# zraorg/ZRA

Hardware: AMD Instinct MI355X
Metric: compress + RA-decompress GiB/s, 16 GiB @ 64 KiB frames, 1/2/4/8 MI355X (higher is better)
Workload: dtype u8

## Files before the change

zra_amd/csrc/zra_decode.hip:

```cpp
#include "zra_dev.h"
#include "zra_kernels.h"

using namespace zra_dev;

namespace {

constexpr int DEC_THREADS = 64;
constexpr int BATCH = 64;
#ifndef ZRA_XWIN
#define ZRA_XWIN 4032
#endif
constexpr u32 XPRE = 64, XWIN = ZRA_XWIN;
constexpr u32 BLOCK_MAX = 128u << 10;

__constant__ u32 c_ll_base[36] = {0,1,2,3,4,5,6,7,8,9,10,11,12,13,14,15,16,18,20,22,24,28,32,40,48,64,128,256,512,1024,2048,4096,8192,16384,32768,65536};
__constant__ u8 c_ll_bits[36] = {0,0,0,0,0,0,0,0,0,0,0,0,0,0,0,0,1,1,1,1,2,2,3,3,4,6,7,8,9,10,11,12,13,14,15,16};
__constant__ u32 c_ml_base[53] = {3,4,5,6,7,8,9,10,11,12,13,14,15,16,17,18,19,20,21,22,23,24,25,26,27,28,29,30,31,32,33,34,
                                  35,37,39,41,43,47,51,59,67,83,99,131,259,515,1027,2051,4099,8195,16387,32771,65539};
__constant__ u8 c_ml_bits[53] = {0,0,0,0,0,0,0,0,0,0,0,0,0,0,0,0,0,0,0,0,0,0,0,0,0,0,0,0,0,0,0,0,
                                 1,1,1,1,2,2,3,3,4,4,5,7,8,9,10,11,12,13,14,15,16};
__constant__ short c_ll_defnorm[36] = {4,3,2,2,2,2,2,2,2,2,2,2,2,1,1,1,2,2,2,2,2,2,2,2,2,3,2,1,1,1,1,1,-1,-1,-1,-1};
__constant__ short c_ml_defnorm[53] = {1,4,3,2,2,2,2,2,2,1,1,1,1,1,1,1,1,1,1,1,1,1,1,1,1,1,1,1,1,1,1,1,
                                       1,1,1,1,1,1,1,1,1,1,1,1,1,1,-1,-1,-1,-1,-1,-1,-1};
__constant__ short c_of_defnorm[29] = {1,1,1,1,1,1,2,2,2,1,1,1,1,1,1,1,1,1,1,1,1,1,1,1,-1,-1,-1,-1,-1};
__constant__ u16 c_huf_t0[16][2] = {{0,0},{0,0},{38,130},{448,128},{556,128},{714,128},{883,128},{897,128},{926,128},{947,128},{1107,128},{1177,128},{1242,128},{1349,128},{1455,128},{722,128}};
__constant__ u16 c_huf_t1[16][2] = {{1,1},{1,1},{1313,74},{1353,74},{1353,74},{1418,74},{1437,74},{1515,75},{1613,75},{1729,77},{2083,81},{2379,87},{2415,93},{2644,106},{2422,124},{1891,145}};

__device__ __forceinline__ u64 mk_seqsym(u32 baseValue, u32 addBits, u32 nbBits, u32 nextBase) {
  return (u64)baseValue | ((u64)addBits << 32) | ((u64)nbBits << 40) | ((u64)nextBase << 48);
}
__device__ __forceinline__ u32 mk_cell(u32 sym, u32 addBits, u32 nbBits, u32 nextBase) {
  return sym | (addBits << 8) | (nbBits << 16) | (nextBase << 20);
}

#ifdef ZRA_SMALL_PROFILE
__device__ unsigned long long zra_small_prof[64];
extern "C" __attribute__((visibility("default"))) void ZraHipDebugReadSmallProfile(unsigned long long* out16, int reset) {
  (void)hipMemcpyFromSymbol(out16, HIP_SYMBOL(zra_small_prof), sizeof(unsigned long long) * 64);
  if (reset) { unsigned long long z[64] = {0}; (void)hipMemcpyToSymbol(HIP_SYMBOL(zra_small_prof), z, sizeof(z)); }
}
#define SPROF(k) { __builtin_amdgcn_s_waitcnt(0); const u64 n_ = __builtin_amdgcn_s_memtime(); if (lane == 0) atomicAdd(&zra_small_prof[k], n_ - spt_); spt_ = n_; }
#define SPROF_T0 u64 spt_ = __builtin_amdgcn_s_memtime();
#define SPROF_RESET spt_ = __builtin_amdgcn_s_memtime();
#else
#define SPROF(k)
#define SPROF_T0
#define SPROF_RESET
#endif
#ifdef ZRA_SMALL_PROFILE
#define PPROF_T0 u64 ppt_ = __builtin_amdgcn_s_memtime();
#define PPROF(k) if (FUSED) { __builtin_amdgcn_s_waitcnt(0); const u64 n_ = __builtin_amdgcn_s_memtime(); if (lane == 0) atomicAdd(&zra_small_prof[k], n_ - ppt_); ppt_ = n_; }
#define LPROF_T0 u64 lpt_ = __builtin_amdgcn_s_memtime();
#define LPROF(k) { __builtin_amdgcn_s_waitcnt(0); const u64 n_ = __builtin_amdgcn_s_memtime(); atomicAdd(&zra_small_prof[k], n_ - lpt_); lpt_ = n_; }
#else
#define PPROF_T0
// ... 495 lines not shown
        if (have) copy_bytes(a.raOut + q.dstOff, a.out + a.outOff[j] + q.srcOff, have, lane, nthreads);
        if (have < q.len) fill_bytes(a.raOut + q.dstOff + have, 0, q.len - have, lane, nthreads);
      }
    }
  }
}

}

namespace {
template <bool FUSED, bool ALL = false>
__device__ __forceinline__ u32 parse_job(const ZraDecodeArgs& a, const u32 j, ParseShared& S, const int lane, u32* ldsT) {
  u32 outcome = 0;
  {
    const u64 so = a.frameOff[(size_t)j * a.offStride], se = a.frameOff[(size_t)j * a.offStride + 1];
    const u8* const src = a.body + so;
    const bool spanOk = se >= so && se <= a.bodySize;
    const u32 srcSize = spanOk ? (u32)(se - so) : 0u;
    u8* const dst = a.out + a.outOff[j];
    const u32 dstCap = a.outCap[j];
    const u32 limit = a.limit ? a.limit[j] : 0xFFFFFFFFu;
    ZraDecFrame* const F = &a.frames[j];
    u32 nBlk = 0; bool bail = false;
    const u32* prevT[3] = {nullptr, nullptr, nullptr};

    auto stage = [&](u8* w, u32 pos) -> u32 {
      const u32 avail = pos < srcSize ? min(srcSize - pos, STAGE_BYTES) : 0u;
      const u32 at = 8u * (u32)lane;
      u64 v = 0;
      if (at + 8 <= avail) v = ld64(src + pos + at);
      else for (u32 k = 0; at + k < avail && k < 8; k++) v |= (u64)src[pos + at + k] << (8 * k);
      *(u64*)(w + at) = v;
      if (lane < 2) *(u64*)(w + STAGE_BYTES + 8 * lane) = 0;
      return avail;
    };
    PPROF_T0
    const u32 startPos = a.round == 0 ? 0u : F->blkPos;
    const u32 staged0 = stage(S.w0, startPos);

    if (lane == 0) {
      S.err = 0; S.frameEnd = 0; S.winPos = startPos; S.winLen = staged0;
      if (a.round == 0) {
        S.produced = 0; S.hufValid = 0; S.llValid = S.mlValid = S.ofValid = 0; S.ofShare = 0;
        S.rep[0] = 1; S.rep[1] = 4; S.rep[2] = 8;
      }
    }
    wsync();
// ... 140 lines not shown
        if (S.err) { S.lateErr = S.err; S.err = 0; S.nbSeq = 0; S.seqTables = 0; }
        if (S.alloc && S.nbSeq) {
          const u64 take = ((u64)S.nbSeq + 3) & ~3ull;
          const u64 at = atomicAdd((unsigned long long*)&a.counters[ZRA_DC_SEQCUR], (unsigned long long)take);
          if (at + take > a.seqCap) S.alloc = 0;
          S.seqBase = at;
        }
      }
      wsync();
      if (ALL && (!S.alloc || nBlk >= a.bpf)) { bail = true; break; }
      if (!S.alloc) {
        if (lane == 0) {
          save_persistent(S.hdrPos, produced0, hv0, hmb0, hns0, hx20);
          if (!FUSED) a.nextActive[atomicAdd(&a.counters[ZRA_DC_NNEXT], 1u)] = j;
        }
        handed = true; outcome = 2;
        wsync();
        break;
      }

      PPROF(10)
      const u32 nbSeq = S.nbSeq, regen = S.litRegen;
      const size_t jb = ALL ? (size_t)j * a.bpf + nBlk : (size_t)j;
      u32* const T = ALL ? a.blkTables + jb * ZRA_DEC_TBL_WORDS : a.tables + (size_t)j * ZRA_DEC_TBL_WORDS;
      if (S.seqTables) {
        for (int kind = 0; kind < 3; kind++) {
          const int k = kind == 0 ? 0 : kind == 1 ? 2 : 1;
          const u32 mode = k == 0 ? (S.seqModes >> 6) : k == 2 ? ((S.seqModes >> 4) & 3) : ((S.seqModes >> 2) & 3);
          if (lane == 0) {
            u32 tl = 0, ms = 0, used = 0;
            seq_table_parse(S, k, mode, sw + S.seqPos, bsize - S.seqPos, &tl, &ms, &used, swLim);
            S.seqPos += used; S.tl = tl; S.ms = ms;
            if (mode == 3) { u32 v = k == 0 ? S.llValid : k == 1 ? S.mlValid : S.ofValid; if (!v) S.err = ZE_CORRUPTION; }
            if (S.err) { S.lateErr = S.err; S.err = 0; }
          }
          wsync();
          PPROF(11)
          if (S.lateErr) break;
          const u32 tl = S.tl, ms = S.ms;
          u32* const G = T + (k == 0 ? ZRA_DEC_TBL_LL : k == 1 ? ZRA_DEC_TBL_ML : ZRA_DEC_TBL_OF);
          if (mode == 1) {
            if (lane == 0) {
              if (k == 2) { G[0] = mk_cell(ms, ms, 0, 0); S.ofShare = (ms > 22) ? 256u : 0u; }
              else G[0] = mk_cell(ms, k == 0 ? c_ll_bits[ms] : c_ml_bits[ms], 0, 0);
              if (FUSED) { u32* const GL = ldsT + (k == 0 ? ZRA_LDS_TBL_LL : k == 1 ? ZRA_LDS_TBL_ML : ZRA_LDS_TBL_OF); GL[0] = G[0]; if (k != 2) GL[1] = k == 0 ? c_ll_base[ms] : c_ml_base[ms]; }
            }
          } else if (mode != 3) {
            build_fse_dtable(S.stage, S.norm, ms, tl, k, S.spread, (u64*)S.w0, S.wnext, lane);
            wsync();
            const u32 words = (k == 2 ? 1u : 2u) << tl;
            if (!FUSED) for (u32 i = lane; i < (1u << tl); i += DEC_THREADS) G[i] = S.stage[k == 2 ? i : 2 * i];
            if (FUSED) { u32* const GL = ldsT + (k == 0 ? ZRA_LDS_TBL_LL : k == 1 ? ZRA_LDS_TBL_ML : ZRA_LDS_TBL_OF); for (u32 i = lane; i < words; i += DEC_THREADS) GL[i] = S.stage[i]; }
            if (k == 2) {
              u32 cnt = 0;
              for (u32 i = lane; i < (1u << tl); i += DEC_THREADS) cnt += (S.stage[i] & 0xFF) > 22;
              cnt = wave_sum(cnt);
              if (lane == 0) S.ofShare = cnt << (8 - tl);
            }
            wsync();
          }
          if (lane == 0 && mode != 3) {
            if (k == 0) { S.llLog = tl; S.llValid = 1; } else if (k == 1) { S.mlLog = tl; S.mlValid = 1; } else { S.ofLog = tl; S.ofValid = 1; }
          }
          if (ALL) {
            if (mode == 3 && prevT[k] && prevT[k] != G) {
              const u32 lg = k == 0 ? S.llLog : k == 1 ? S.mlLog : S.ofLog;
              for (u32 i = lane; i < (1u << lg); i += DEC_THREADS) G[i] = prevT[k][i];
            }
            prevT[k] = G;
          }
          wsync();
          PPROF(12)
        }
      }
// ... 417 lines not shown
    u32 nbBytes = bc >> 3; int r = UNFINISHED;
    if (ptr < nbBytes) { nbBytes = ptr; r = ENDOFBUFFER; }
    ptr -= nbBytes; bc -= nbBytes * 8; c = fetch(ptr);
    return r;
  }
  __device__ __forceinline__ void reload_quiet(bool wide, const u8* pad) {
    const u32 nb = bc <= 64 ? min(bc >> 3, ptr) : 0u;
    ptr -= nb; bc -= nb * 8;
    const u64 v = RING ? fetch(ptr) : ld64(wide ? base + ptr : pad);
    c = nb ? v : c;
  }
};
typedef ZdsT<false> Zds;

}

namespace {
template <bool LDSTAB>
__device__ __forceinline__ void chain_body(const ZraDecodeArgs& a, u32* const ldsTabs, u32* const baseLL, u32* const baseML, u32* const ldsRings = nullptr) {
  const int lane = threadIdx.x;
  const u32 nPend = a.counters[ZRA_DC_NPENDING];
  bool have = false, drained = false;
  ZraDecFrame* F = nullptr;
  const u32* T = nullptr;
  u64* sq = nullptr;
  ZdsT<LDSTAB> br; br.c = 0; br.bc = 0; br.ptr = 0; br.base = nullptr; br.ring = nullptr; br.rLo = 0;
  br.lim = a.body + a.bodySize; br.pf = make_uint4(0, 0, 0, 0); br.pfState = 0; br.pfAge = 0;
  if (LDSTAB) br.ring = (u8*)(ldsRings + (u32)lane * CHAIN_RING_WORDS);
  u32 sLL = 0, sOF = 0, sML = 0, rep0 = 1, rep1 = 4, rep2 = 8;
  u32 i = 0, nbSeq = 0, outPos = 0, litPos = 0, outCap = 0, regen = 0, produced0 = 0, limit = 0;
  u32 longMode = 0, err = 0, jErr = 0xFFFFFFFFu, valid = 0, validOut = 0, validLit = 0, truncated = 0;
  u64 q0 = 0, q1 = 0, q2 = 0;
  u32 eL = 0, eM = 0, eO = 0;
  bool wide = false; const u8* pad = nullptr;
  bool fresh = false; u32 freshJob = 0;
  const u16* const cells16 = (const u16*)ldsTabs + (size_t)lane * ZRA_DEC_TBL_WORDS;
  u32 logLL = 0, logML = 0, logOF = 0;
  auto fetch_cells = [&]() {
    if (LDSTAB) { eL = cells16[ZRA_DEC_TBL_LL + sLL]; eM = cells16[ZRA_DEC_TBL_ML + sML]; eO = cells16[ZRA_DEC_TBL_OF + sOF]; }
    else { eL = T[ZRA_DEC_TBL_LL + sLL]; eM = T[ZRA_DEC_TBL_ML + sML]; eO = T[ZRA_DEC_TBL_OF + sOF]; }
  };
  auto c_code = [&](u32 e) -> u32 { return e & 63u; };
  auto c_sbits = [&](u32 e, u32 lg) -> u32 { if (LDSTAB) return lg - (31u - (u32)__builtin_clz(e >> 6)); return (e >> 16) & 0xF; };
  auto c_sbase = [&](u32 e, u32 lg) -> u32 {
    if (LDSTAB) { const u32 v = e >> 6, hb = 31u - (u32)__builtin_clz(v); return (v ^ (1u << hb)) << (lg - hb); }
    return e >> 20;
  };
  baseLL[lane] = lane < 36 ? c_ll_base[lane] | (LDSTAB ? (u32)c_ll_bits[lane] << 24 : 0u) : 0u;
  baseML[lane] = lane < 53 ? c_ml_base[lane] | (LDSTAB ? (u32)c_ml_bits[lane] << 24 : 0u) : 0u;
  wsync();
  if (LDSTAB && (u32)lane >= ZRA_CHAIN_LDS_FRAMES) drained = true;

  auto finish = [&]() {
    { const u32 r = valid & 3u, b = valid - r;
      if (r >= 1) sq[b] = q0;
      if (r >= 2) sq[b + 1] = q1;
      if (r >= 3) sq[b + 2] = q2; }
    if (!err && !truncated) {
      if (regen - litPos > outCap - outPos) err = ZE_DSTSIZE_TOOSMALL;
    }
    F->chainErr = err; F->nSeqValid = valid; F->seqOut = validOut; F->seqLit = validLit; F->truncated = truncated;
    F->repOut[0] = rep0; F->repOut[1] = rep1; F->repOut[2] = rep2;
    have = false;
  };

  for (;;) {
    const u64 want = __ballot(!have && !drained);
    if (want) {
      u32 base = 0;
      const u32 cnt = (u32)__builtin_popcountll(want);
      if (lane == (int)__builtin_ctzll(want)) base = atomicAdd(&a.counters[ZRA_DC_QCHAIN], cnt);
      base = bcast_u32(base, (u32)__builtin_ctzll(want));
      if (!have && !drained) {
        const u32 idx = base + (u32)__builtin_popcountll(want & ((1ull << lane) - 1ull));
        if (idx >= nPend) drained = true;
        else {
          const u32 j = a.pending[idx];
          const size_t gj = frame_of(a, j);
          F = &a.frames[j];
          T = a.tables + (size_t)j * ZRA_DEC_TBL_WORDS;
          const u8* const blk = a.body + a.frameOff[gj * a.offStride] + F->bpos;
          nbSeq = F->nbSeq; regen = F->litRegen; produced0 = F->produced; longMode = F->longMode;
          outCap = a.outCap[gj] - produced0;
          limit = a.limit ? a.limit[gj] : 0xFFFFFFFFu;
          sq = a.seqs + F->seqBase;
          rep0 = F->rep[0]; rep1 = F->rep[1]; rep2 = F->rep[2];
          i = 0; outPos = 0; litPos = 0; err = 0; jErr = 0xFFFFFFFFu; valid = 0; validOut = 0; validLit = 0; truncated = 0;
          have = true; br.rLo = 0; br.pfState = 0;
          if (F->hufErr) { err = ZE_CORRUPTION; nbSeq = 0; finish(); }
          else if (F->lateErr) { err = F->lateErr; nbSeq = 0; finish(); }
          else if (nbSeq) {
            if (!br.init(blk + F->seqPos, F->bsize - F->seqPos)) { err = ZE_CORRUPTION; finish(); }
            else {
              logLL = F->llLog; logOF = F->ofLog; logML = F->mlLog;
              sLL = br.read(logLL); br.reload();
              sOF = br.read(logOF); br.reload();
              sML = br.read(logML); br.reload();
              wide = F->bsize - F->seqPos >= 8;
              pad = a.body + a.frameOff[gj * a.offStride];
              if (LDSTAB) { fresh = true; freshJob = j; } else fetch_cells();
            }
          }
        }
      }
    }
    if (LDSTAB) {
      u64 nm = __ballot(fresh);
      while (nm) {
        const u32 l = (u32)__builtin_ctzll(nm); nm &= nm - 1;
        const u32 jj = bcast_u32(freshJob, l);
        const uint4* const g4 = (const uint4*)(a.tables + (size_t)jj * ZRA_DEC_TBL_WORDS);
        uint2* const d2 = (uint2*)((u16*)ldsTabs + (size_t)l * ZRA_DEC_TBL_WORDS);
        const ZraDecFrame* const Fj = &a.frames[jj];
        const u32 lgL = Fj->llLog, lgM = Fj->mlLog, lgO = Fj->ofLog;
        for (u32 i = (u32)lane; i < ZRA_DEC_TBL_WORDS / 4; i += DEC_THREADS) {
          const uint4 q = g4[i];
          const u32 lg = 4 * i < ZRA_DEC_TBL_ML ? lgL : 4 * i < ZRA_DEC_TBL_OF ? lgM : lgO;
          auto pk = [&](u32 x) -> u32 { const u32 nb = min((x >> 16) & 0xFu, lg); return (x & 63u) | (((1u << (lg - nb)) | ((x >> 20) >> nb)) << 6); };
          d2[i] = make_uint2(pk(q.x) | (pk(q.y) << 16), pk(q.z) | (pk(q.w) << 16));
        }
      }
      if (__ballot(fresh)) wsync();
      if (fresh) { fetch_cells(); fresh = false; }
    }
    if (!__ballot(have)) break;

    if (have) {
      bool go = true;
      if (LDSTAB) { br.ring_guard(); br.ring_advance(); }
      if (i >= nbSeq) {
        if (!err && nbSeq && !longMode && br.reload() < Zds::COMPLETED) err = ZE_CORRUPTION;
        finish(); go = false;
      } else if (longMode) {
        if (br.reload() > Zds::COMPLETED) {
          if (jErr == 0xFFFFFFFFu || i <= jErr + 4) err = ZE_CORRUPTION;
          finish(); go = false;
        } else if (jErr != 0xFFFFFFFFu && i > jErr + 4) { finish(); go = false; }
      }
      if (go) {
        u32 ll = baseLL[c_code(eL)], ml = baseML[c_code(eM)], off;
        const u32 ofBits = LDSTAB ? c_code(eO) : (eO >> 8) & 0xFF, mlBits = LDSTAB ? ml >> 24 : (eM >> 8) & 0xFF, llBits = LDSTAB ? ll >> 24 : (eL >> 8) & 0xFF;
        if (LDSTAB) { ll &= 0xFFFFFFu; ml &= 0xFFFFFFu; }
        bool badOff = false;
        if (ofBits > 1) {
          off = ((1u << ofBits) - 3u) + br.read_fast(ofBits);
          if (a.bpf > 1 && off >= ZRA_REP_MARK_LO) badOff = true;
          rep2 = rep1; rep1 = rep0; rep0 = off;
        } else {
          const u32 ll0 = (ll == 0);
          if (ofBits == 0) {
            if (!ll0) off = rep0;
            else { off = rep1; rep1 = rep0; rep0 = off; }
          } else {
            const u32 idx = 1 + ll0 + br.read_fast(1);
            u32 t = idx == 3 ? rep0 - 1 : idx == 1 ? rep1 : rep2;
            t += !t;
            if (idx != 1) rep2 = rep1;
            rep1 = rep0; rep0 = off = t;
          }
        }
        if (mlBits) ml += br.read_fast(mlBits);
        if (llBits + mlBits + ofBits >= 57 - (9 + 9 + 8)) br.reload();
        if (llBits) ll += br.read_fast(llBits);
        sLL = c_sbase(eL, logLL) + br.read(c_sbits(eL, logLL));
        sML = c_sbase(eM, logML) + br.read(c_sbits(eM, logML));
        sOF = c_sbase(eO, logOF) + br.read(c_sbits(eO, logOF));
        fetch_cells();
        if (!longMode) br.reload_quiet(wide, pad);
        if (jErr == 0xFFFFFFFFu) {
          u32 e = 0;
          if (ll + ml > outCap - outPos) e = ZE_DSTSIZE_TOOSMALL;
          else if (ll > regen - litPos) e = ZE_CORRUPTION;
          else if (badOff || (off > produced0 + outPos + ll && !(a.bpf > 1 && off >= ZRA_REP_MARK_LO))) e = ZE_CORRUPTION;
          if (e) { jErr = i; err = e; if (!longMode) finish(); }
          else {
            const u64 qv = (u64)ll | ((u64)ml << 18) | ((u64)min(off, 0x0FFFFFFFu) << 36);
            const u32 slot = i & 3u;
            if (slot == 0) q0 = qv; else if (slot == 1) q1 = qv; else if (slot == 2) q2 = qv;
            else { uint4* d4 = (uint4*)(sq + (i - 3)); d4[0] = make_uint4((u32)q0, (u32)(q0 >> 32), (u32)q1, (u32)(q1 >> 32)); d4[1] = make_uint4((u32)q2, (u32)(q2 >> 32), (u32)qv, (u32)(qv >> 32)); }
            outPos += ll + ml; litPos += ll;
            valid = i + 1; validOut = outPos; validLit = litPos;
            if (produced0 + outPos >= limit) { truncated = 1; finish(); }
          }
        }
        i++;
      }
    }
  }
}
}

extern "C" __global__ void __launch_bounds__(DEC_THREADS)
zra_dec_chain_kernel(ZraDecodeArgs a) {
  __shared__ u32 baseLL[64], baseML[64];
  chain_body<false>(a, nullptr, baseLL, baseML);
}
extern "C" __global__ void __launch_bounds__(DEC_THREADS)
zra_dec_chain_lds_kernel(ZraDecodeArgs a) {
  extern __shared__ u32 chainLds[];
  chain_body<true>(a, chainLds + 128, chainLds, chainLds + 64, chainLds + 128 + ZRA_CHAIN_LDS_FRAMES * (ZRA_DEC_TBL_WORDS / 2));
}

namespace {
struct __attribute__((aligned(16))) ExecShared {
  union {
    u8 slot[BATCH][64];
    u8 win[XPRE + XWIN];
  };
  u32 endAt[BATCH];
  u32 matchAt[BATCH];
  u32 job;
};
}

#ifdef ZRA_DEC_PROFILE
__device__ unsigned long long zra_dec_prof[16];
#define XCNT(k, v) { if (lane == 0) atomicAdd(&zra_dec_prof[k], (unsigned long long)(v)); }
#define XTIME(k) { __builtin_amdgcn_s_waitcnt(0); const u64 n_ = __builtin_amdgcn_s_memtime(); if (lane == 0) atomicAdd(&zra_dec_prof[k], n_ - xpt_); xpt_ = n_; }
extern "C" __attribute__((visibility("default"))) void ZraHipDebugReadDecProfile(unsigned long long* out16, int reset) {
  (void)hipMemcpyFromSymbol(out16, HIP_SYMBOL(zra_dec_prof), sizeof(unsigned long long) * 16);
  if (reset) { unsigned long long z[16] = {0}; (void)hipMemcpyToSymbol(HIP_SYMBOL(zra_dec_prof), z, sizeof(z)); }
}
#else
// ... 642 lines not shown
```

zra_amd/csrc/zra_engine.h:

```cpp
#pragma once
#include <hip/hip_runtime.h>
#include <cstdint>
#include <cstddef>
#include <vector>
#include "zra_kernels.h"

namespace zra_eng {

struct Status { int zra; int zstd; };
enum : int { kSuccess = 0, kZStdError = 1, kVersionLow = 2, kHeaderInvalid = 3, kHeaderIncomplete = 4, kOutOfBounds = 5,
             kOutputTooSmall = 6, kCompressedTooLarge = 7, kFrameSizeMismatch = 8 };
inline Status ok() { return {kSuccess, 0}; }
inline Status zerr(int code) { return {kZStdError, (int)(int8_t)code}; }

struct DevBuf {
  void* p = nullptr; size_t cap = 0;
  bool reserve(size_t n);
  void release();
  template <typename T> T* as() const { return (T*)p; }
};

uint64_t scratch_bytes_in_use();

struct HeaderInfo {
// ... 109 lines not shown

  Status compare_archives(const uint8_t* dA, size_t sizeA, const uint8_t* dB, size_t sizeB, uint32_t mode, uint64_t offset, uint64_t size,
                          size_t stagingBytes, uint64_t* hRanges, size_t rangeCap, uint64_t* nRanges, uint64_t* differingBytes);
  void compare_stats(uint64_t out[8]) const { for (int i = 0; i < 8; i++) out[i] = cstats_[i]; }
  void compare_sizes(uint64_t out[2]) const { out[0] = cmpSizes_[0]; out[1] = cmpSizes_[1]; }
  double compare_ms() const { return compareMs_; }

  Status compress_host(const uint8_t* hIn, size_t n, uint8_t* hOut, size_t* outSize, int level, uint32_t frameSize, bool checksum);
  Status compress_frames_host(const uint8_t* hIn, size_t n, uint8_t* hBody, std::vector<uint64_t>& sizes, size_t* bodySize,
                              int level, uint32_t frameSize, bool checksum);
  Status decode_host(const uint8_t* hSpan, size_t spanSize, const std::vector<uint64_t>& starts, const std::vector<uint64_t>& ends,
                     uint32_t frameSize, uint64_t total, uint8_t* hOut, size_t skip, size_t size, bool wholeArchive = false);
  Status decode_host_pipelined(const uint8_t* hSpan, const std::vector<uint64_t>& starts, const std::vector<uint64_t>& ends,
                               uint32_t frameSize, uint64_t total, uint8_t* hOut, bool* fallBack);

  void set_ra_verify_whole_frames(bool on) { raVerifyWholeFrames_ = on; }
  bool ra_verify_whole_frames() const { return raVerifyWholeFrames_; }
  int device() const { return device_; }
  int num_cus() const { return numCUs_; }

 private:
  Engine() = default;
  int device_ = 0, numCUs_ = 0;
  hipStream_t stream_ = nullptr;
  hipEvent_t ev0_ = nullptr, ev1_ = nullptr, evWait_ = nullptr;
  double lastKernelMs_ = 0;
  std::vector<uint64_t> mfTele_;
  const uint64_t* mfTeleDev_ = nullptr;
  double kstats_[6] = {0, 0, 0, 0, 0, 0};
  double dstats_[8] = {0, 0, 0, 0, 0, 0, 0, 0};
  std::vector<hipEvent_t> stageEv_; size_t stageEvNext_ = 0;
  hipEvent_t stage_event();
  Status launch_stages(uint64_t nJobs, const struct ZraDecodeArgs& a, const struct ZraDecodeArgs& mid, uint32_t nFrames, bool blockPass, hipEvent_t se[5]);
  Status launch_chain(uint64_t nJobs, const struct ZraDecodeArgs& mid, hipEvent_t after);
  Status decode_sequential_tail(const struct ZraDecodeArgs& a, const uint64_t* dFrameOff, uint32_t offStride, const uint64_t* dOutOff, uint32_t first,
                                uint32_t nFrames, uint32_t maxFrameBytes, uint64_t seqTotal);
  Status upload_jobs(const std::vector<uint64_t>& frameOff, const std::vector<uint64_t>& outOff, const std::vector<uint32_t>& expect);
  Status read_fixed_header(const uint8_t* dArc, size_t arcSize, HeaderInfo* h);
  uint64_t* pinned_tuples(size_t nTuples);
  void reset_decode_stats() { kstats_[4] = kstats_[5] = 0; for (auto& d : dstats_) d = 0; }
  static float elapsed_ms(hipEvent_t e0, hipEvent_t e1) { float ms = 0; if (hipEventElapsedTime(&ms, e0, e1) != hipSuccess) { ms = 0; (void)hipGetLastError(); } return ms; }
  bool call_events() {
    for (auto& ev : evCall_) if (!ev && hipEventCreate(&ev) != hipSuccess) { ev = nullptr; (void)hipGetLastError(); return false; }
    return true;
  }
  void free_scratch();
// ... 56 lines not shown
```

zra_amd/csrc/zra_engine.hip:

```cpp
#include "zra_host.h"
#include "zra_dev.h"
#include "zra_format.h"
#include <algorithm>
#include <atomic>

extern "C" __global__ void zra_dec_parse_kernel(ZraDecodeArgs a);
extern "C" __global__ void zra_dec_huf_kernel(ZraDecodeArgs a);
extern "C" __global__ void zra_dec_chain_kernel(ZraDecodeArgs a);
extern "C" __global__ void zra_dec_chain_lds_kernel(ZraDecodeArgs a);
extern "C" __global__ void zra_dec_exec_kernel(ZraDecodeArgs a);
extern "C" __global__ void zra_dec_parse_all_kernel(ZraDecodeArgs a);
extern "C" __global__ void zra_dec_exec_all_kernel(ZraDecodeArgs a);
extern "C" __global__ void zra_ra_small_kernel(ZraDecodeArgs a, uint32_t* bail, const uint32_t* expect, uint32_t jobBase, unsigned long long* result);

using namespace zra_dev;

namespace zra_fmt {
uint32_t crc32(uint32_t crc, const void* data, size_t n) {
  static uint32_t T[8][256];
  static bool init = false;
  if (!init) {
    for (uint32_t i = 0; i < 256; i++) {
      uint32_t c = i;
      for (int k = 0; k < 8; k++) c = (c & 1) ? (0xEDB88320u ^ (c >> 1)) : (c >> 1);
// ... 73 lines not shown
  using namespace zra_fmt;
  if (rd32(b + 8) != kZraMagic || rd16(b + 12) > kVersion) return kHeaderInvalid;
  h->version = rd16(b + 12);
  h->size = rd32(b + 4) + 8;
  h->uncompressedSize = rd64(b + 18);
  h->frameSize = rd32(b + 30);
  h->metaOffset = (uint32_t)kFixedSize;
  h->metaSize = rd32(b + 34);
  h->seekTableOffset = h->metaOffset + h->metaSize;
  h->seekTableSize = rd32(b + 26) * (uint32_t)kEntrySize;
  if (h->version != 1) return kVersionLow;
  return 0;
}

Status Engine::create(Engine** out, int device) {
  int n = 0;
  if (hipGetDeviceCount(&n) != hipSuccess || n <= 0 || device < 0 || device >= n) return zerr(1);
  HIPCHK(hipSetDevice(device));
  Engine* e = new Engine();
  e->device_ = device;
  hipDeviceProp_t prop;
  if (hipGetDeviceProperties(&prop, device) != hipSuccess) { delete e; return zerr(1); }
  e->numCUs_ = prop.multiProcessorCount;
  if (hipStreamCreateWithFlags(&e->stream_, hipStreamNonBlocking) != hipSuccess) { delete e; return zerr(1); }
  {
    int lo = 0, hi = 0;
    if (hipDeviceGetStreamPriorityRange(&lo, &hi) == hipSuccess && hi != lo) {
      if (hipStreamCreateWithPriority(&e->stream2_, hipStreamNonBlocking, hi) != hipSuccess) { delete e; return zerr(1); }
    } else if (hipStreamCreateWithFlags(&e->stream2_, hipStreamNonBlocking) != hipSuccess) { delete e; return zerr(1); }
  }
  if (hipEventCreate(&e->ev0_) != hipSuccess || hipEventCreate(&e->ev1_) != hipSuccess ||
      hipEventCreateWithFlags(&e->evWait_, hipEventDisableTiming) != hipSuccess) { delete e; return zerr(1); }
  for (auto& ev : e->evR_) if (hipEventCreate(&ev) != hipSuccess) { delete e; return zerr(1); }
  *out = e;
  return ok();
}

void Engine::free_scratch() {
  for (DevBuf* b : {&raPlan_, &raLimit_, &raPieceBase_, &raPieces_, &decFrames_, &decTables_, &decLists_, &decCounters_, &decLits_, &decSeqs_, &roundN_, &status_,
                    &produced_, &frameMeta_, &frameOff_, &outOff_, &expect_, &result_, &stage_, &qmeta_, &encScan_, &hostIn_, &hostOut_, &seqScratch_, &mfFlags_, &decBlkRecs_, &decBlkTables_, &decBlkLists_})
    b->release();
  for (auto& x : encCtx_) for (DevBuf* b : {&x.tables, &x.seqs, &x.lits, &x.work, &x.slots, &x.misc, &x.ck, &x.sizes, &x.rec}) b->release();
  for (DevBuf* b : {&upd_.plan, &upd_.packed, &upd_.encSizes, &upd_.frames, &upd_.table, &upd_.copies}) b->release();
  for (DevBuf* b : {&vfy_.plan, &vfy_.faults, &srch_.tables, &srch_.list, &msrch_.tables, &msrch_.list, &cmp_.flags, &cmp_.tables, &cmp_.list}) b->release();
}

// ... 20 lines not shown
  for (auto& ev : evR_) if (ev) (void)hipEventDestroy(ev);
  for (auto ev : evCall_) if (ev) (void)hipEventDestroy(ev);
  if (ev0_) (void)hipEventDestroy(ev0_);
  if (ev1_) (void)hipEventDestroy(ev1_);
  if (evWait_) (void)hipEventDestroy(evWait_);
  if (stream_) (void)hipStreamDestroy(stream_);
}

Status Engine::sync() { HIPCHK(hipSetDevice(device_)); HIPCHK(hipStreamSynchronize(stream_)); HIPCHK(hipStreamSynchronize(stream2_)); return ok(); }

Status Engine::wait_stream(hipStream_t producer) {
  HIPCHK(hipSetDevice(device_));
  HIPCHK(hipEventRecord(evWait_, producer));
  HIPCHK(hipStreamWaitEvent(stream_, evWait_, 0));
  HIPCHK(hipStreamWaitEvent(stream2_, evWait_, 0));
  return ok();
}

Status Engine::decode_scratch(ZraDecodeArgs& a, uint32_t maxFrameBytes) {
  const uint32_t n = a.nFrames;
  const uint64_t perFrame = std::min<uint64_t>((uint64_t)maxFrameBytes + 16, (128u << 10) + 16);
  const uint64_t litCap = std::max<uint64_t>((uint64_t)n * perFrame / 2, 1u << 20);
  const uint64_t seqCap = std::max<uint64_t>((uint64_t)n * perFrame * 3 / 32, 1u << 20);
  if (!decFrames_.reserve((size_t)n * sizeof(ZraDecFrame)) || !decTables_.reserve((size_t)n * ZRA_DEC_TBL_WORDS * 4) ||
      !decLists_.reserve((size_t)n * 16 + 64) || !decCounters_.reserve(ZRA_DC_WORDS * 4 + 64) || !decLits_.reserve(litCap + 64) ||
      !decSeqs_.reserve(seqCap * 8 + 64) || !status_.reserve((size_t)n * 4) || !produced_.reserve((size_t)n * 4) ||
      !frameMeta_.reserve((size_t)n * 8) || !result_.reserve(64))
    return zerr(64 );
  uint32_t* listA = decLists_.as<uint32_t>();
  a.pending = listA + 2 * (size_t)n; a.hufJobs = listA + 3 * (size_t)n;
  a.counters = decCounters_.as<uint32_t>();
  a.frames = decFrames_.as<ZraDecFrame>(); a.tables = decTables_.as<uint32_t>();
  a.lits = decLits_.as<uint8_t>(); a.litCap = litCap; a.seqs = decSeqs_.as<uint64_t>(); a.seqCap = seqCap;
  a.status = status_.as<uint32_t>(); a.produced = produced_.as<uint32_t>(); a.frameMeta = frameMeta_.as<uint32_t>();
  return ok();
}

Status Engine::decode_small(const ZraDecodeArgs& a0, const uint32_t* dExpect, uint32_t maxFrameBytes, uint32_t jobBase, unsigned long long* hResult, uint32_t* bailed) {
  ZraDecodeArgs a = a0;
  const uint32_t n = a.nFrames;
  RaTrace trace{"    small", 12};
  { Status st = decode_scratch(a, maxFrameBytes); if (st.zra) return st; }
  trace.mark("scratch");
  a.active = nullptr; a.nActive = n; a.round = 0; a.nextActive = decLists_.as<uint32_t>();
  if (!decCountersClean_) HIPCHK(hipMemsetAsync(a.counters, 0, ZRA_DC_WORDS * 4, stream_));
  decCountersClean_ = false;
  uint32_t* dBail = (uint32_t*)(result_.as<uint8_t>() + 8);
  HIPCHK(hipEventRecord(ev0_, stream_));
  hipLaunchKernelGGL(zra_ra_small_kernel, dim3(n), dim3(192), 0, stream_, a, dBail, dExpect, jobBase, result_.as<unsigned long long>());
  HIPCHK(hipEventRecord(ev1_, stream_));
  trace.mark("launched");
  unsigned long long two[2] = {~0ull, ~0ull};
  HIPCHK(hipMemcpyAsync(two, result_.p, 16, hipMemcpyDeviceToHost, stream_));
  trace.mark("queued rest");
  HIPCHK(hipStreamSynchronize(stream_));
  trace.mark("sync");
  HIPCHK(hipGetLastError());
  if (hipMemsetAsync(a.counters, 0, ZRA_DC_WORDS * 4, stream_) == hipSuccess) decCountersClean_ = true;
  two[1] = 0xFFFFFFFFull - (two[1] & 0xFFFFFFFFull);
  *bailed = (uint32_t)two[1];
  if (!*bailed) *hResult = two[0];
  float ms = 0;
  if (hipEventElapsedTime(&ms, ev0_, ev1_) == hipSuccess) { lastKernelMs_ = ms; kstats_[4] += ms; kstats_[5] += 1; dstats_[5] += ms; dstats_[6] += 1; }
  return ok();
}

hipEvent_t Engine::stage_event() {
  if (stageEvNext_ == stageEv_.size()) { hipEvent_t e = nullptr; if (hipEventCreate(&e) != hipSuccess) return nullptr; stageEv_.push_back(e); }
  return stageEv_[stageEvNext_++];
}

Status Engine::launch_chain(uint64_t nJobs, const ZraDecodeArgs& mid, hipEvent_t after) {
  constexpr uint32_t chainWaves = 2;
  static const uint32_t chainLdsMin = (uint32_t)zra_env::env_int("ZRA_DEC_CHAIN_LDS_MIN", numCUs_ * 96);
  static const int chainLdsMode = zra_env::env_int("ZRA_DEC_CHAIN_LDS", 1);
  const uint32_t gridChain = (uint32_t)std::min<uint64_t>((nJobs + 63) / 64, (uint64_t)numCUs_ * chainWaves);
  if (chainLdsMode != 0 && nJobs >= chainLdsMin) {
    if (!pipeStreams_[1]) { if (hipStreamCreateWithFlags(&pipeStreams_[1], hipStreamNonBlocking) != hipSuccess) { pipeStreams_[1] = nullptr; (void)hipGetLastError(); } }
    const size_t ldsBytes = (128 + (size_t)ZRA_CHAIN_LDS_FRAMES * (ZRA_DEC_TBL_WORDS / 2 + ZRA_CHAIN_RING_WORDS)) * 4;
    if (pipeStreams_[1] && !chainLdsAttr_) {
      if (hipFuncSetAttribute((const void*)zra_dec_chain_lds_kernel, hipFuncAttributeMaxDynamicSharedMemorySize, (int)ldsBytes) == hipSuccess) chainLdsAttr_ = 1;
      else { chainLdsAttr_ = -1; (void)hipGetLastError(); }
    }
    if (pipeStreams_[1] && chainLdsAttr_ > 0) {
      hipEvent_t eJoin = stage_event(); if (!eJoin) return zerr(1);
      HIPCHK(hipStreamWaitEvent(pipeStreams_[1], after, 0));
      hipLaunchKernelGGL(zra_dec_chain_lds_kernel, dim3((uint32_t)numCUs_), dim3(64), ldsBytes, pipeStreams_[1], mid);
      HIPCHK(hipEventRecord(eJoin, pipeStreams_[1]));
      if (chainLdsMode != 2) hipLaunchKernelGGL(zra_dec_chain_kernel, dim3(gridChain), dim3(64), 0, stream_, mid);
      HIPCHK(hipStreamWaitEvent(stream_, eJoin, 0));
      return ok();
    }
  }
  hipLaunchKernelGGL(zra_dec_chain_kernel, dim3(gridChain), dim3(64), 0, stream_, mid);
  return ok();
}

Status Engine::launch_stages(uint64_t nJobs, const ZraDecodeArgs& a, const ZraDecodeArgs& mid, uint32_t nFrames, bool blockPass, hipEvent_t se[5]) {
  for (int k = 0; k < 5; k++) { se[k] = stage_event(); if (!se[k]) return zerr(1); }
  const uint32_t gridParse = (uint32_t)std::min<uint64_t>(nFrames, (uint64_t)numCUs_ * decOccParse_);
  const uint32_t gridHuf = (uint32_t)std::min<uint64_t>((nJobs + ZRA_HUF_FRAMES - 1) / ZRA_HUF_FRAMES, (uint64_t)numCUs_ * decOccHuf_);
  const uint32_t gridExec = (uint32_t)std::min<uint64_t>(nFrames, (uint64_t)numCUs_ * decOccExec_);
// ... 13 lines not shown
  ZraDecodeArgs a = a0;
  const uint32_t n = a.nFrames;
  { Status st = decode_scratch(a, maxFrameBytes); if (st.zra) return st; }
  decCountersClean_ = false;
  uint32_t* listA = decLists_.as<uint32_t>(); uint32_t* listB = listA + n;
  if (!decOccParse_) {
    HIPCHK(hipOccupancyMaxActiveBlocksPerMultiprocessor(&decOccParse_, zra_dec_parse_kernel, 64, 0));
    HIPCHK(hipOccupancyMaxActiveBlocksPerMultiprocessor(&decOccExec_, zra_dec_exec_kernel, 64, 0));
    HIPCHK(hipOccupancyMaxActiveBlocksPerMultiprocessor(&decOccHuf_, zra_dec_huf_kernel, 64, 0));
    decOccParse_ = std::max(1, decOccParse_); decOccExec_ = std::max(1, decOccExec_); decOccHuf_ = std::max(1, decOccHuf_);
  }
  HIPCHK(hipEventRecord(ev0_, stream_));
  constexpr uint32_t aheadCap = 16;
  if (!roundN_.reserve(4 * (aheadCap + 2) + 64)) return zerr(64);
  static const int fmbEnv = zra_env::env_int("ZRA_DEC_FMB", 1);
  static const uint32_t fmbMin = (uint32_t)zra_env::env_int("ZRA_DEC_FMB_MIN", 64);
  const uint32_t bpf = (uint32_t)(((uint64_t)maxFrameBytes + ZRA_FMB_BLOCK - 1) / ZRA_FMB_BLOCK);
  bool fmb = fmbEnv != 0 && bpf >= 2 && maxFrameBytes <= (64u << 20) && n >= fmbMin && (uint64_t)n * bpf < (1ull << 30);
  uint32_t nRest = n;
  if (fmb) {
    const uint64_t nb = (uint64_t)n * bpf;
    const uint64_t litAll = std::max<uint64_t>((uint64_t)n * ((uint64_t)maxFrameBytes + 16) / 2, 1u << 20);
    const uint64_t seqAll = std::max<uint64_t>((uint64_t)n * ((uint64_t)maxFrameBytes + 16) * 3 / 32, 1u << 20);
    if (!decBlkRecs_.reserve((size_t)nb * sizeof(ZraDecFrame)) || !decBlkTables_.reserve((size_t)nb * ZRA_DEC_TBL_WORDS * 4) ||
        !decBlkLists_.reserve((size_t)(2 * nb + n) * 4 + 64) || !decLits_.reserve(litAll + 64) || !decSeqs_.reserve(seqAll * 8 + 64)) {
      (void)hipGetLastError();
      fmb = false;
    }
    a.lits = decLits_.as<uint8_t>(); a.seqs = decSeqs_.as<uint64_t>();
    if (fmb) {
      ZraDecodeArgs x = a;
      x.bpf = bpf; x.blkRecs = decBlkRecs_.as<ZraDecFrame>(); x.blkTables = decBlkTables_.as<uint32_t>();
      uint32_t* bl = decBlkLists_.as<uint32_t>();
      x.pending = bl; x.hufJobs = bl + nb; x.execList = bl + 2 * nb;
      x.litCap = litAll; x.seqCap = seqAll;
      x.active = nullptr; x.nActive = n; x.round = 0; x.nActivePtr = nullptr; x.nextActive = listA;
      HIPCHK(hipMemsetAsync(x.counters, 0, ZRA_DC_WORDS * 4, stream_));
      ZraDecodeArgs y = x; y.frames = x.blkRecs; y.tables = x.blkTables;
      hipEvent_t se[5];
      { Status st = launch_stages(nb, x, y, n, true, se); if (st.zra) return st; }
      uint32_t back = 0;
      HIPCHK(hipMemcpyAsync(&back, x.counters + ZRA_DC_NNEXT, 4, hipMemcpyDeviceToHost, stream_));
      HIPCHK(hipStreamSynchronize(stream_));
      HIPCHK(hipGetLastError());
      for (int k = 0; k < 4; k++) { float m = 0; if (hipEventElapsedTime(&m, se[k], se[k + 1]) == hipSuccess) dstats_[k] += m; }
      dstats_[4] += 1;
      stageEvNext_ = 0;
      nRest = back;
    }
  }
  auto run_rounds = [&](ZraDecodeArgs& x, uint32_t nActive, const uint32_t* active, uint32_t round, uint32_t* lA, uint32_t* lB, uint32_t ahead) -> Status {
    uint32_t* const dN = roundN_.as<uint32_t>();
    while (nActive) {
      const uint32_t burst = std::max(1u, std::min(ahead, aheadCap));
      hipEvent_t se[aheadCap][5];
// ... 205 lines not shown
```

zra_amd/csrc/zra_kernels.h:

```cpp
#pragma once
#include <stdint.h>
#include <stddef.h>

#ifndef ZRA_HUF_FRAMES
#define ZRA_HUF_FRAMES 2
#endif
#define ZRA_DEC_TBL_LL 0u
#define ZRA_DEC_TBL_ML 512u
#define ZRA_DEC_TBL_OF 1024u
#define ZRA_DEC_TBL_WORDS 1280u
#define ZRA_LDS_TBL_LL 0u
#define ZRA_LDS_TBL_ML 1024u
#define ZRA_LDS_TBL_OF 2048u
#define ZRA_LDS_TBL_WORDS 2304u
#define ZRA_CHAIN_LDS_FRAMES 59u
#define ZRA_CHAIN_RING_WORDS 36u

struct ZraDecFrame {
  uint32_t blkPos, produced, done;
  uint32_t hufValid, hufMaxBits, hufNSym, hufX2;
  uint32_t llValid, mlValid, ofValid, llLog, mlLog, ofLog, ofShare;
  uint32_t rep[3];
  uint32_t fcsLo, fcsHi, fcsHave, hasChecksum, bigWindow;
  uint32_t bpos, bsize, blast;
  uint32_t litKind, litRegen, litArg;
  uint32_t litStreams, streamOff[4], streamLen[4];
  uint32_t hufErr, lateErr;
  uint32_t nbSeq, seqPos, longMode;
  uint64_t litBase, seqBase;
  uint32_t chainErr, nSeqValid, seqOut, seqLit, truncated;
  uint32_t repOut[3];
  uint32_t nBlk, endPos, parseTrunc, pad1_;
  alignas(8) uint8_t weights[256];
// ... 19 lines not shown

struct ZraDecodeArgs {
  const uint8_t* body;
  uint64_t bodySize;
  const uint64_t* frameOff;
  uint32_t offStride;
  uint8_t* out;
  const uint64_t* outOff;
  const uint32_t* outCap;
  uint32_t nFrames;
  const uint32_t* limit;
  const uint32_t* pieceBase;
  const ZraRaPiece* pieces;
  uint8_t* raOut;
  const uint32_t* active;
  uint32_t nActive;
  const uint32_t* nActivePtr;
  uint32_t round;
  uint32_t* counters;
  uint32_t* nextActive;
  uint32_t* pending;
  uint32_t* hufJobs;
  ZraDecFrame* frames;
  uint32_t* tables;
  uint8_t* lits; uint64_t litCap;
  uint64_t* seqs; uint64_t seqCap;
  uint32_t* status;
  uint32_t* produced;
  uint32_t* frameMeta;
  uint32_t debugSkip;
  uint32_t bpf;
  ZraDecFrame* blkRecs;
  uint32_t* blkTables;
  uint32_t* execList;
};
#define ZRA_DC_QPARSE 0
#define ZRA_DC_QCHAIN 1
#define ZRA_DC_QEXEC 2
#define ZRA_DC_NPENDING 3
#define ZRA_DC_NNEXT 4
#define ZRA_DC_NHUF 5
#define ZRA_DC_QHUF 10
#define ZRA_DC_LITCUR 6
#define ZRA_DC_SEQCUR 8
#define ZRA_DC_NEXEC 11
#define ZRA_DC_QEXECALL 12
#define ZRA_DC_WORDS 16

struct ZraEncParams {
  uint32_t windowLog, chainLog, hashLog, searchLog, minMatch, targetLength, strategy;
  uint32_t blockSize;
};

#define ZRA_OPT_NUM 4096u
struct ZraOptCell { int32_t price; uint32_t off, mlen, litlen, rep[3]; };
struct ZraOptMatch { uint32_t off, len; };
// ... 112 lines not shown
```

Measured before the change: 20.32.

## Store FSE decode tables as packed 16-bit cells and size chain grid from L2

Global FSE decode tables change from 32-bit cells to the packed 16-bit form the LDS chain path already used. The parse kernel packs each cell when it writes it, so the chain kernel copies tables into LDS directly instead of repacking them. The non-LDS path decodes the same compact format and masks the next states. This halves table memory traffic and footprint, and the chain grid size is now derived from XCD count and L2 capacity so more jobs' tables fit in cache, at the cost of extra clz work in the global path.

```diff
diff --git a/zra_amd/csrc/zra_decode.hip b/zra_amd/csrc/zra_decode.hip
--- a/zra_amd/csrc/zra_decode.hip
+++ b/zra_amd/csrc/zra_decode.hip
@@ -31,6 +31,10 @@
 }
 __device__ __forceinline__ u32 mk_cell(u32 sym, u32 addBits, u32 nbBits, u32 nextBase) {
   return sym | (addBits << 8) | (nbBits << 16) | (nextBase << 20);
+}
+__device__ __forceinline__ u16 cell16(u32 cell4, u32 tableLog) {
+  const u32 nb = (cell4 >> 16) & 0xFu;
+  return (u16)((cell4 & 63u) | (((1u << (tableLog - nb)) | ((cell4 >> 20) >> nb)) << 6));
 }
 
 #ifdef ZRA_SMALL_PROFILE
@@ -572,7 +576,7 @@
     const u32 limit = a.limit ? a.limit[j] : 0xFFFFFFFFu;
     ZraDecFrame* const F = &a.frames[j];
     u32 nBlk = 0; bool bail = false;
-    const u32* prevT[3] = {nullptr, nullptr, nullptr};
+    const u16* prevT[3] = {nullptr, nullptr, nullptr};
 
     auto stage = [&](u8* w, u32 pos) -> u32 {
       const u32 avail = pos < srcSize ? min(srcSize - pos, STAGE_BYTES) : 0u;
@@ -759,7 +763,7 @@
       PPROF(10)
       const u32 nbSeq = S.nbSeq, regen = S.litRegen;
       const size_t jb = ALL ? (size_t)j * a.bpf + nBlk : (size_t)j;
-      u32* const T = ALL ? a.blkTables + jb * ZRA_DEC_TBL_WORDS : a.tables + (size_t)j * ZRA_DEC_TBL_WORDS;
+      u16* const T = ALL ? a.blkTables + jb * ZRA_DEC_TBL_CELLS : a.tables + (size_t)j * ZRA_DEC_TBL_CELLS;
       if (S.seqTables) {
         for (int kind = 0; kind < 3; kind++) {
           const int k = kind == 0 ? 0 : kind == 1 ? 2 : 1;
@@ -775,18 +779,19 @@
           PPROF(11)
           if (S.lateErr) break;
           const u32 tl = S.tl, ms = S.ms;
-          u32* const G = T + (k == 0 ? ZRA_DEC_TBL_LL : k == 1 ? ZRA_DEC_TBL_ML : ZRA_DEC_TBL_OF);
+          u16* const G = T + (k == 0 ? ZRA_DEC_TBL_LL : k == 1 ? ZRA_DEC_TBL_ML : ZRA_DEC_TBL_OF);
           if (mode == 1) {
             if (lane == 0) {
-              if (k == 2) { G[0] = mk_cell(ms, ms, 0, 0); S.ofShare = (ms > 22) ? 256u : 0u; }
-              else G[0] = mk_cell(ms, k == 0 ? c_ll_bits[ms] : c_ml_bits[ms], 0, 0);
-              if (FUSED) { u32* const GL = ldsT + (k == 0 ? ZRA_LDS_TBL_LL : k == 1 ? ZRA_LDS_TBL_ML : ZRA_LDS_TBL_OF); GL[0] = G[0]; if (k != 2) GL[1] = k == 0 ? c_ll_base[ms] : c_ml_base[ms]; }
+              const u32 c4 = mk_cell(ms, k == 2 ? ms : k == 0 ? c_ll_bits[ms] : c_ml_bits[ms], 0, 0);
+              G[0] = cell16(c4, 0);
+              if (k == 2) S.ofShare = (ms > 22) ? 256u : 0u;
+              if (FUSED) { u32* const GL = ldsT + (k == 0 ? ZRA_LDS_TBL_LL : k == 1 ? ZRA_LDS_TBL_ML : ZRA_LDS_TBL_OF); GL[0] = c4; if (k != 2) GL[1] = k == 0 ? c_ll_base[ms] : c_ml_base[ms]; }
             }
           } else if (mode != 3) {
             build_fse_dtable(S.stage, S.norm, ms, tl, k, S.spread, (u64*)S.w0, S.wnext, lane);
             wsync();
             const u32 words = (k == 2 ? 1u : 2u) << tl;
-            if (!FUSED) for (u32 i = lane; i < (1u << tl); i += DEC_THREADS) G[i] = S.stage[k == 2 ? i : 2 * i];
+            if (!FUSED) for (u32 i = lane; i < (1u << tl); i += DEC_THREADS) G[i] = cell16(S.stage[k == 2 ? i : 2 * i], tl);
             if (FUSED) { u32* const GL = ldsT + (k == 0 ? ZRA_LDS_TBL_LL : k == 1 ? ZRA_LDS_TBL_ML : ZRA_LDS_TBL_OF); for (u32 i = lane; i < words; i += DEC_THREADS) GL[i] = S.stage[i]; }
             if (k == 2) {
               u32 cnt = 0;
@@ -1250,7 +1255,7 @@
   const u32 nPend = a.counters[ZRA_DC_NPENDING];
   bool have = false, drained = false;
   ZraDecFrame* F = nullptr;
-  const u32* T = nullptr;
+  const u16* T = nullptr;
   u64* sq = nullptr;
   ZdsT<LDSTAB> br; br.c = 0; br.bc = 0; br.ptr = 0; br.base = nullptr; br.ring = nullptr; br.rLo = 0;
   br.lim = a.body + a.bodySize; br.pf = make_uint4(0, 0, 0, 0); br.pfState = 0; br.pfAge = 0;
@@ -1262,20 +1267,17 @@
   u32 eL = 0, eM = 0, eO = 0;
   bool wide = false; const u8* pad = nullptr;
   bool fresh = false; u32 freshJob = 0;
-  const u16* const cells16 = (const u16*)ldsTabs + (size_t)lane * ZRA_DEC_TBL_WORDS;
+  const u16* const cells16 = (const u16*)ldsTabs + (size_t)lane * ZRA_DEC_TBL_CELLS;
   u32 logLL = 0, logML = 0, logOF = 0;
   auto fetch_cells = [&]() {
-    if (LDSTAB) { eL = cells16[ZRA_DEC_TBL_LL + sLL]; eM = cells16[ZRA_DEC_TBL_ML + sML]; eO = cells16[ZRA_DEC_TBL_OF + sOF]; }
-    else { eL = T[ZRA_DEC_TBL_LL + sLL]; eM = T[ZRA_DEC_TBL_ML + sML]; eO = T[ZRA_DEC_TBL_OF + sOF]; }
+    const u16* const C = LDSTAB ? cells16 : T;
+    eL = C[ZRA_DEC_TBL_LL + sLL]; eM = C[ZRA_DEC_TBL_ML + sML]; eO = C[ZRA_DEC_TBL_OF + sOF];
   };
   auto c_code = [&](u32 e) -> u32 { return e & 63u; };
-  auto c_sbits = [&](u32 e, u32 lg) -> u32 { if (LDSTAB) return lg - (31u - (u32)__builtin_clz(e >> 6)); return (e >> 16) & 0xF; };
-  auto c_sbase = [&](u32 e, u32 lg) -> u32 {
-    if (LDSTAB) { const u32 v = e >> 6, hb = 31u - (u32)__builtin_clz(v); return (v ^ (1u << hb)) << (lg - hb); }
-    return e >> 20;
-  };
-  baseLL[lane] = lane < 36 ? c_ll_base[lane] | (LDSTAB ? (u32)c_ll_bits[lane] << 24 : 0u) : 0u;
-  baseML[lane] = lane < 53 ? c_ml_base[lane] | (LDSTAB ? (u32)c_ml_bits[lane] << 24 : 0u) : 0u;
+  auto c_sbits = [&](u32 e, u32 lg) -> u32 { return lg - (31u - (u32)__builtin_clz(e >> 6)); };
+  auto c_sbase = [&](u32 e, u32 lg) -> u32 { const u32 v = e >> 6, hb = 31u - (u32)__builtin_clz(v); return (v ^ (1u << hb)) << (lg - hb); };
+  baseLL[lane] = lane < 36 ? c_ll_base[lane] | ((u32)c_ll_bits[lane] << 24) : 0u;
+  baseML[lane] = lane < 53 ? c_ml_base[lane] | ((u32)c_ml_bits[lane] << 24) : 0u;
   wsync();
   if (LDSTAB && (u32)lane >= ZRA_CHAIN_LDS_FRAMES) drained = true;
 
@@ -1306,7 +1308,7 @@
           const u32 j = a.pending[idx];
           const size_t gj = frame_of(a, j);
           F = &a.frames[j];
-          T = a.tables + (size_t)j * ZRA_DEC_TBL_WORDS;
+          T = a.tables + (size_t)j * ZRA_DEC_TBL_CELLS;
           const u8* const blk = a.body + a.frameOff[gj * a.offStride] + F->bpos;
           nbSeq = F->nbSeq; regen = F->litRegen; produced0 = F->produced; longMode = F->longMode;
           outCap = a.outCap[gj] - produced0;
@@ -1337,16 +1339,9 @@
       while (nm) {
         const u32 l = (u32)__builtin_ctzll(nm); nm &= nm - 1;
         const u32 jj = bcast_u32(freshJob, l);
-        const uint4* const g4 = (const uint4*)(a.tables + (size_t)jj * ZRA_DEC_TBL_WORDS);
-        uint2* const d2 = (uint2*)((u16*)ldsTabs + (size_t)l * ZRA_DEC_TBL_WORDS);
-        const ZraDecFrame* const Fj = &a.frames[jj];
-        const u32 lgL = Fj->llLog, lgM = Fj->mlLog, lgO = Fj->ofLog;
-        for (u32 i = (u32)lane; i < ZRA_DEC_TBL_WORDS / 4; i += DEC_THREADS) {
-          const uint4 q = g4[i];
-          const u32 lg = 4 * i < ZRA_DEC_TBL_ML ? lgL : 4 * i < ZRA_DEC_TBL_OF ? lgM : lgO;
-          auto pk = [&](u32 x) -> u32 { const u32 nb = min((x >> 16) & 0xFu, lg); return (x & 63u) | (((1u << (lg - nb)) | ((x >> 20) >> nb)) << 6); };
-          d2[i] = make_uint2(pk(q.x) | (pk(q.y) << 16), pk(q.z) | (pk(q.w) << 16));
-        }
+        const uint4* const g4 = (const uint4*)(a.tables + (size_t)jj * ZRA_DEC_TBL_CELLS);
+        uint4* const d4 = (uint4*)((u16*)ldsTabs + (size_t)l * ZRA_DEC_TBL_CELLS);
+        for (u32 i = (u32)lane; i < ZRA_DEC_TBL_CELLS / 8; i += DEC_THREADS) d4[i] = g4[i];
       }
       if (__ballot(fresh)) wsync();
       if (fresh) { fetch_cells(); fresh = false; }
@@ -1367,8 +1362,8 @@
       }
       if (go) {
         u32 ll = baseLL[c_code(eL)], ml = baseML[c_code(eM)], off;
-        const u32 ofBits = LDSTAB ? c_code(eO) : (eO >> 8) & 0xFF, mlBits = LDSTAB ? ml >> 24 : (eM >> 8) & 0xFF, llBits = LDSTAB ? ll >> 24 : (eL >> 8) & 0xFF;
-        if (LDSTAB) { ll &= 0xFFFFFFu; ml &= 0xFFFFFFu; }
+        const u32 ofBits = c_code(eO), mlBits = ml >> 24, llBits = ll >> 24;
+        ll &= 0xFFFFFFu; ml &= 0xFFFFFFu;
         bool badOff = false;
         if (ofBits > 1) {
           off = ((1u << ofBits) - 3u) + br.read_fast(ofBits);
@@ -1393,6 +1388,7 @@
         sLL = c_sbase(eL, logLL) + br.read(c_sbits(eL, logLL));
         sML = c_sbase(eM, logML) + br.read(c_sbits(eM, logML));
         sOF = c_sbase(eO, logOF) + br.read(c_sbits(eO, logOF));
+        if (!LDSTAB) { sLL &= ~(~0u << logLL); sML &= ~(~0u << logML); sOF &= ~(~0u << logOF); }
         fetch_cells();
         if (!longMode) br.reload_quiet(wide, pad);
         if (jErr == 0xFFFFFFFFu) {
@@ -1426,7 +1422,7 @@
 extern "C" __global__ void __launch_bounds__(DEC_THREADS)
 zra_dec_chain_lds_kernel(ZraDecodeArgs a) {
   extern __shared__ u32 chainLds[];
-  chain_body<true>(a, chainLds + 128, chainLds, chainLds + 64, chainLds + 128 + ZRA_CHAIN_LDS_FRAMES * (ZRA_DEC_TBL_WORDS / 2));
+  chain_body<true>(a, chainLds + 128, chainLds, chainLds + 64, chainLds + 128 + ZRA_CHAIN_LDS_FRAMES * (ZRA_DEC_TBL_CELLS / 2));
 }
 
 namespace {
diff --git a/zra_amd/csrc/zra_engine.h b/zra_amd/csrc/zra_engine.h
--- a/zra_amd/csrc/zra_engine.h
+++ b/zra_amd/csrc/zra_engine.h
@@ -155,6 +155,7 @@
  private:
   Engine() = default;
   int device_ = 0, numCUs_ = 0;
+  uint32_t chainGrid_ = 0;
   hipStream_t stream_ = nullptr;
   hipEvent_t ev0_ = nullptr, ev1_ = nullptr, evWait_ = nullptr;
   double lastKernelMs_ = 0;
diff --git a/zra_amd/csrc/zra_engine.hip b/zra_amd/csrc/zra_engine.hip
--- a/zra_amd/csrc/zra_engine.hip
+++ b/zra_amd/csrc/zra_engine.hip
@@ -119,6 +119,14 @@
   hipDeviceProp_t prop;
   if (hipGetDeviceProperties(&prop, device) != hipSuccess) { delete e; return zerr(1); }
   e->numCUs_ = prop.multiProcessorCount;
+  {
+    int xcds = 0;
+    if (hipDeviceGetAttribute(&xcds, hipDeviceAttributeNumberOfXccs, device) != hipSuccess || xcds < 1) { (void)hipGetLastError(); xcds = std::max(1, e->numCUs_ / 32); }
+    const uint64_t l2 = prop.l2CacheSize > 0 ? (uint64_t)prop.l2CacheSize : (4ull << 20);
+    const uint64_t jobsPerXcd = l2 * ZRA_CHAIN_L2_OVERSUB_X8 / 8 / (ZRA_DEC_TBL_CELLS * 2);
+    const uint64_t wgs = (uint64_t)xcds * jobsPerXcd / 64;
+    e->chainGrid_ = (uint32_t)std::min<uint64_t>(std::max<uint64_t>(wgs, (uint64_t)e->numCUs_), (uint64_t)e->numCUs_ * 4);
+  }
   if (hipStreamCreateWithFlags(&e->stream_, hipStreamNonBlocking) != hipSuccess) { delete e; return zerr(1); }
   {
     int lo = 0, hi = 0;
@@ -185,7 +193,7 @@
   const uint64_t perFrame = std::min<uint64_t>((uint64_t)maxFrameBytes + 16, (128u << 10) + 16);
   const uint64_t litCap = std::max<uint64_t>((uint64_t)n * perFrame / 2, 1u << 20);
   const uint64_t seqCap = std::max<uint64_t>((uint64_t)n * perFrame * 3 / 32, 1u << 20);
-  if (!decFrames_.reserve((size_t)n * sizeof(ZraDecFrame)) || !decTables_.reserve((size_t)n * ZRA_DEC_TBL_WORDS * 4) ||
+  if (!decFrames_.reserve((size_t)n * sizeof(ZraDecFrame)) || !decTables_.reserve((size_t)n * ZRA_DEC_TBL_CELLS * 2) ||
       !decLists_.reserve((size_t)n * 16 + 64) || !decCounters_.reserve(ZRA_DC_WORDS * 4 + 64) || !decLits_.reserve(litCap + 64) ||
       !decSeqs_.reserve(seqCap * 8 + 64) || !status_.reserve((size_t)n * 4) || !produced_.reserve((size_t)n * 4) ||
       !frameMeta_.reserve((size_t)n * 8) || !result_.reserve(64))
@@ -193,7 +201,7 @@
   uint32_t* listA = decLists_.as<uint32_t>();
   a.pending = listA + 2 * (size_t)n; a.hufJobs = listA + 3 * (size_t)n;
   a.counters = decCounters_.as<uint32_t>();
-  a.frames = decFrames_.as<ZraDecFrame>(); a.tables = decTables_.as<uint32_t>();
+  a.frames = decFrames_.as<ZraDecFrame>(); a.tables = decTables_.as<uint16_t>();
   a.lits = decLits_.as<uint8_t>(); a.litCap = litCap; a.seqs = decSeqs_.as<uint64_t>(); a.seqCap = seqCap;
   a.status = status_.as<uint32_t>(); a.produced = produced_.as<uint32_t>(); a.frameMeta = frameMeta_.as<uint32_t>();
   return ok();
@@ -234,13 +242,12 @@
 }
 
 Status Engine::launch_chain(uint64_t nJobs, const ZraDecodeArgs& mid, hipEvent_t after) {
-  constexpr uint32_t chainWaves = 2;
   static const uint32_t chainLdsMin = (uint32_t)zra_env::env_int("ZRA_DEC_CHAIN_LDS_MIN", numCUs_ * 96);
   static const int chainLdsMode = zra_env::env_int("ZRA_DEC_CHAIN_LDS", 1);
-  const uint32_t gridChain = (uint32_t)std::min<uint64_t>((nJobs + 63) / 64, (uint64_t)numCUs_ * chainWaves);
+  const uint32_t gridChain = (uint32_t)std::min<uint64_t>((nJobs + 63) / 64, (uint64_t)chainGrid_);
   if (chainLdsMode != 0 && nJobs >= chainLdsMin) {
     if (!pipeStreams_[1]) { if (hipStreamCreateWithFlags(&pipeStreams_[1], hipStreamNonBlocking) != hipSuccess) { pipeStreams_[1] = nullptr; (void)hipGetLastError(); } }
-    const size_t ldsBytes = (128 + (size_t)ZRA_CHAIN_LDS_FRAMES * (ZRA_DEC_TBL_WORDS / 2 + ZRA_CHAIN_RING_WORDS)) * 4;
+    const size_t ldsBytes = (128 + (size_t)ZRA_CHAIN_LDS_FRAMES * (ZRA_DEC_TBL_CELLS / 2 + ZRA_CHAIN_RING_WORDS)) * 4;
     if (pipeStreams_[1] && !chainLdsAttr_) {
       if (hipFuncSetAttribute((const void*)zra_dec_chain_lds_kernel, hipFuncAttributeMaxDynamicSharedMemorySize, (int)ldsBytes) == hipSuccess) chainLdsAttr_ = 1;
       else { chainLdsAttr_ = -1; (void)hipGetLastError(); }
@@ -300,7 +307,7 @@
     const uint64_t nb = (uint64_t)n * bpf;
     const uint64_t litAll = std::max<uint64_t>((uint64_t)n * ((uint64_t)maxFrameBytes + 16) / 2, 1u << 20);
     const uint64_t seqAll = std::max<uint64_t>((uint64_t)n * ((uint64_t)maxFrameBytes + 16) * 3 / 32, 1u << 20);
-    if (!decBlkRecs_.reserve((size_t)nb * sizeof(ZraDecFrame)) || !decBlkTables_.reserve((size_t)nb * ZRA_DEC_TBL_WORDS * 4) ||
+    if (!decBlkRecs_.reserve((size_t)nb * sizeof(ZraDecFrame)) || !decBlkTables_.reserve((size_t)nb * ZRA_DEC_TBL_CELLS * 2) ||
         !decBlkLists_.reserve((size_t)(2 * nb + n) * 4 + 64) || !decLits_.reserve(litAll + 64) || !decSeqs_.reserve(seqAll * 8 + 64)) {
       (void)hipGetLastError();
       fmb = false;
@@ -308,7 +315,7 @@
     a.lits = decLits_.as<uint8_t>(); a.seqs = decSeqs_.as<uint64_t>();
     if (fmb) {
       ZraDecodeArgs x = a;
-      x.bpf = bpf; x.blkRecs = decBlkRecs_.as<ZraDecFrame>(); x.blkTables = decBlkTables_.as<uint32_t>();
+      x.bpf = bpf; x.blkRecs = decBlkRecs_.as<ZraDecFrame>(); x.blkTables = decBlkTables_.as<uint16_t>();
       uint32_t* bl = decBlkLists_.as<uint32_t>();
       x.pending = bl; x.hufJobs = bl + nb; x.execList = bl + 2 * nb;
       x.litCap = litAll; x.seqCap = seqAll;
diff --git a/zra_amd/csrc/zra_kernels.h b/zra_amd/csrc/zra_kernels.h
--- a/zra_amd/csrc/zra_kernels.h
+++ b/zra_amd/csrc/zra_kernels.h
@@ -8,7 +8,10 @@
 #define ZRA_DEC_TBL_LL 0u
 #define ZRA_DEC_TBL_ML 512u
 #define ZRA_DEC_TBL_OF 1024u
-#define ZRA_DEC_TBL_WORDS 1280u
+#define ZRA_DEC_TBL_CELLS 1280u
+#ifndef ZRA_CHAIN_L2_OVERSUB_X8
+#define ZRA_CHAIN_L2_OVERSUB_X8 20u
+#endif
 #define ZRA_LDS_TBL_LL 0u
 #define ZRA_LDS_TBL_ML 1024u
 #define ZRA_LDS_TBL_OF 2048u
@@ -74,7 +77,7 @@
   uint32_t* pending;
   uint32_t* hufJobs;
   ZraDecFrame* frames;
-  uint32_t* tables;
+  uint16_t* tables;
   uint8_t* lits; uint64_t litCap;
   uint64_t* seqs; uint64_t seqCap;
   uint32_t* status;
@@ -83,7 +86,7 @@
   uint32_t debugSkip;
   uint32_t bpf;
   ZraDecFrame* blkRecs;
-  uint32_t* blkTables;
+  uint16_t* blkTables;
   uint32_t* execList;
 };
 #define ZRA_DC_QPARSE 0
```

Result: no change. 20.34, median of 5 (+0.1%).
